# zeehu/generative_ranking_recommender

Measured on NVIDIA B200. Metric: RQ-KMeans vectors/sec per iteration (512-d, [128,128,256]), higher is better.
Workload: dtype 3xTF32 distance (fp32 accumulate), fp16 auction, fp32 centroids

## Files before the change

generative_ranking_recommender_b200/csrc/auction.cu:

```cuda
#include "common.cuh"

namespace rqk {

constexpr int AUC_W = 256;
constexpr int AUC_HALF = AUC_W / 2;
constexpr int AUC_NBUF = 3;
constexpr int AUC_BPL = AUC_W / 32;
constexpr int AUC_NW = 16;
constexpr int AUC_THREADS = AUC_NW * 32;
constexpr int AUC_BASE_CTAS = 296;
constexpr int AUC_MAX_CTAS = 1024;
constexpr int AUC_MAX_JOBS_PER_CTA = 65024;
constexpr int AUC_MIN_TILES_PER_CTA = 2;
constexpr int AUC_COLD_SHIFT = 8;
constexpr int AUC_MIN_KEY = 0x0400;
constexpr int AUC_SUB = 4096;
constexpr int AUC_QCAP = 256;
constexpr int AUC_SAMPLE_MAX = 8192;
constexpr int AUC_SEG_CAP = 256;
constexpr int AUC_KH = 128;
constexpr int AUC_SAMPLE_THREADS = 512;

enum { MODE_HIST = 0, MODE_BID = 1, MODE_DONE = 2 };

__device__ __forceinline__ void pdl_launch_dependents() { asm volatile("griddepcontrol.launch_dependents;" ::: "memory"); }
__device__ __forceinline__ void pdl_wait() { asm volatile("griddepcontrol.wait;" ::: "memory"); }

struct AuctionState {
    int mode;
    int counter;
    int rounds;
    int done;
    int ff_pending;
    int frozen_exit;
    int passes;
    int cold_passes;
    int window_misses;
    unsigned int eps_bits;
    unsigned int smax_bits, smin_bits;
    int need_sample;
    int error;
    int use_list;
    int force_scan;
    int list_passes;
    int sink[4];
    int branch[4];
    int pad_[4];
};

struct AuctionPtrs {
    AuctionState* st;
    __half* cost;
    short* owner;
    __half* sown;
    unsigned int* hist_g;
    unsigned int* above_g;
    unsigned int* gap_g;
    unsigned int* n_with;
    unsigned int* n_viol;
    unsigned int* tie_total;
    int* win_base;
    int* win_hbase;
    int* win_nlo;
    int* win_shift;
    int* tkey;
    int* take;
    int* tprev;
    int* miss_run;
    unsigned int* tieprefix;
    unsigned short* hist_cta;
    unsigned int* seg_list;
    unsigned int* seg_cnt;
    int* list_ok;
    unsigned int* rank_off;
    unsigned int* ticket;
    int* res_pass;
    unsigned int* above_cta;
    unsigned int* gap_cta;
    int* unres_g;
};

static inline int auction_tile_cols(int K) { return K <= 128 ? 128 : 64; }

static inline int auction_grid(long long N, int K) {
    long long tiles = ceil_div<long long>(N, auction_tile_cols(K));
    long long g = ceil_div<long long>(tiles, AUC_MIN_TILES_PER_CTA);
    const char* e = getenv("RQK_AUCTION_GRID");
    const int cap = (e && atoi(e) >= 1 && atoi(e) <= AUC_BASE_CTAS) ? atoi(e) : AUC_BASE_CTAS;
    if (g > cap) g = cap;
    long long g16 = ceil_div<long long>(N, AUC_MAX_JOBS_PER_CTA);
    if (g < g16) g = g16;
    if (g < 1) g = 1;
    return (int)g;
}

static inline int auction_spc(long long N, int K) {
    const int J = auction_tile_cols(K), G = auction_grid(N, K);
    const long long tiles = ceil_div<long long>(N, J);
    const long long len = ceil_div<long long>(tiles, G) * J;
    return (int)ceil_div<long long>(len, AUC_SUB);
}

static inline size_t auction_ws_layout(long long N, long long ld, int K, AuctionPtrs* p, char* base,
                                       size_t* reduce_off = nullptr, size_t* tie_total_off = nullptr) {
    int G = auction_grid(N, K);
    size_t off = 0;
    auto take_ = [&](size_t bytes) { size_t o = off; off += align256(bytes); return o; };
    size_t o_st = take_(sizeof(AuctionState));
    size_t o_cost = take_((size_t)ld * 2);
    size_t o_own = take_((size_t)ld * 2);
    size_t o_sown = take_((size_t)ld * 2);
    size_t o_hist = take_(((size_t)K * AUC_W + 2 * K + 2) * 4);
    size_t o_tt = take_((size_t)K * 4);
    size_t o_wb = take_((size_t)K * 4);
    size_t o_whb = take_((size_t)K * 4);
    size_t o_wnl = take_((size_t)K * 4);
    size_t o_ws = take_((size_t)K * 4);
    size_t o_tk = take_((size_t)K * 4);
    size_t o_take = take_((size_t)K * 4);
    size_t o_tprev = take_((size_t)K * 4);
    size_t o_mr = take_((size_t)K * 4);
    size_t o_tp = take_((size_t)G * K * 4);
    size_t o_hc = take_((size_t)G * K * AUC_W * 2);
    const size_t nseg = (size_t)G * auction_spc(N, K);
    size_t o_sl = take_(nseg * K * AUC_SEG_CAP * 4);
    size_t o_sc = take_(nseg * K * 4);
    size_t o_lo = take_(4);
    size_t o_ro = take_((size_t)K * 4);
    size_t o_tk2 = take_(4);
    size_t o_rp = take_((size_t)K * 4);
    size_t o_ac = take_((size_t)G * K * 4);
    size_t o_gc = take_((size_t)G * K * 4);
    size_t o_ug = take_(16);
    if (reduce_off) *reduce_off = o_hist;
    if (tie_total_off) *tie_total_off = o_tt;
    if (p) {
        p->st = (AuctionState*)(base + o_st);
        p->cost = (__half*)(base + o_cost);
        p->owner = (short*)(base + o_own);
        p->sown = (__half*)(base + o_sown);
        p->hist_g = (unsigned int*)(base + o_hist);
        p->above_g = p->hist_g + (size_t)K * AUC_W;
        p->gap_g = p->above_g + K;
        p->n_with = p->gap_g + K;
        p->n_viol = p->n_with + 1;
        p->tie_total = (unsigned int*)(base + o_tt);
        p->win_base = (int*)(base + o_wb);
        p->win_hbase = (int*)(base + o_whb);
        p->win_nlo = (int*)(base + o_wnl);
        p->win_shift = (int*)(base + o_ws);
        p->tkey = (int*)(base + o_tk);
        p->take = (int*)(base + o_take);
        p->tprev = (int*)(base + o_tprev);
        p->miss_run = (int*)(base + o_mr);
        p->tieprefix = (unsigned int*)(base + o_tp);
        p->hist_cta = (unsigned short*)(base + o_hc);
        p->seg_list = (unsigned int*)(base + o_sl);
        p->seg_cnt = (unsigned int*)(base + o_sc);
        p->list_ok = (int*)(base + o_lo);
        p->rank_off = (unsigned int*)(base + o_ro);
        p->ticket = (unsigned int*)(base + o_tk2);
        p->res_pass = (int*)(base + o_rp);
        p->above_cta = (unsigned int*)(base + o_ac);
        p->gap_cta = (unsigned int*)(base + o_gc);
        p->unres_g = (int*)(base + o_ug);
    }
    return off;
}

__global__ void auction_init_kernel(AuctionPtrs p, long long ld, int K, const unsigned int* minmax_keys, int force_scan) {
    long long i = (long long)blockIdx.x * blockDim.x + threadIdx.x;
    long long stride = (long long)gridDim.x * blockDim.x;
    for (long long j = i; j < ld; j += stride) {
        p.cost[j] = __ushort_as_half(0);
        p.owner[j] = -1;
    }
    for (long long j = i; j < (long long)K * AUC_W + 2 * K + 2; j += stride) p.hist_g[j] = 0;
    for (long long j = i; j < K; j += stride) {
        p.win_base[j] = 0;
        p.win_hbase[j] = AUC_HALF;
        p.win_nlo[j] = AUC_HALF;
        p.win_shift[j] = AUC_COLD_SHIFT;
        p.tkey[j] = -1;
        p.take[j] = 0;
        p.tprev[j] = -1;
        p.miss_run[j] = 0;
        p.rank_off[j] = 0;
        p.res_pass[j] = -1;
    }
    if (i == 0) {
        AuctionState s;
        memset(&s, 0, sizeof(s));
        s.mode = MODE_HIST;
        s.need_sample = 1;
        s.force_scan = force_scan;
        *p.list_ok = 1;
        *p.ticket = 0;
        p.unres_g[0] = 0;
// ... 139 lines not shown
        atomicAdd(&sink[5], 1);
        int nb2 = base + nlo, span = hbase - nb2, nshift = 0;
        while ((span >> nshift) > AUC_W) ++nshift;
        p.win_base[w] = nb2;
        p.win_hbase[w] = nb2 + AUC_HALF;
        p.win_nlo[w] = AUC_HALF;
        p.win_shift[w] = nshift;
        p.tkey[w] = -1;
        atomicAdd(unresolved, 1);
        atomicAdd(miss, 1);
    } else if (lane == 0) {
        const int run = p.miss_run[w];
        const bool is_above = ab >= (unsigned long long)need;
        int nb = is_above ? (shift == 0 ? hbase + (AUC_W - nlo) : base + (AUC_W << shift)) : base - (AUC_W << shift);
        atomicAdd(&sink[(shift != 0 || run >= 2 || nb < AUC_MIN_KEY || nb > 65536 - AUC_W) ? 7 : 6], 1);
        if (shift != 0 || run >= 2 || nb < AUC_MIN_KEY || nb > 65536 - AUC_W) {
            p.win_base[w] = 0;
            p.win_hbase[w] = AUC_HALF;
            p.win_nlo[w] = AUC_HALF;
            p.win_shift[w] = AUC_COLD_SHIFT;
            p.miss_run[w] = 0;
        } else {
            p.win_base[w] = nb;
            p.win_hbase[w] = nb + AUC_HALF;
            p.win_nlo[w] = AUC_HALF;
            p.miss_run[w] = run + 1;
        }
        p.tkey[w] = -1;
        atomicAdd(unresolved, 1);
        if (shift == 0) atomicAdd(miss, 1);
    }
}

__device__ __noinline__ void auction_resolve_body(AuctionPtrs p, long long N, int K, long long jpw, int expect) {
    __shared__ int s_unresolved, s_miss;
    __shared__ AuctionState s;
    __shared__ unsigned long long s_nwith_g, s_nviol_g;
    const int tid = threadIdx.x, lane = tid & 31, warp = tid >> 5;
    const int NT = blockDim.x, NWARPS = NT >> 5;
    if (tid == 0) { s = *p.st; s_unresolved = 0; s_miss = 0; s_nwith_g = *p.n_with; s_nviol_g = *p.n_viol; }
    __syncthreads();
    if (s.mode == MODE_DONE || (expect >= 0 && s.mode != expect)) return;
    const bool was_bid = (s.mode == MODE_BID);

    bool finished = false, jump = false;
    if (was_bid) {
        const BidOutcome o = bid_outcome(s.counter, s_nwith_g, s_nviol_g, N);
        finished = o.finished;
        jump = o.jump;
    }
    if (finished) {
        __syncthreads();
        if (tid == 0) {
            bool normal = (s_nwith_g == (unsigned long long)N);
            s.rounds = normal ? s.counter + 1 : 1002;
            s.frozen_exit = normal ? 0 : 1;
            s.mode = MODE_DONE;
            s.done = 1;
            s.passes += 1;
            if (s.use_list) s.list_passes += 1;
            *p.st = s;
        }
        return;
    }

    const long long need = jpw + 1;
    if (was_bid) {
// ... 9 lines not shown
        if (tid == 0) s_unresolved = 1;
    } else if (!jump) {
        unsigned int hn[AUC_BPL];
#pragma unroll
        for (int i = 0; i < AUC_BPL; ++i) hn[i] = (warp < K) ? __ldcg(p.hist_g + warp * AUC_W + lane * AUC_BPL + i) : 0u;
        for (int w = warp; w < K; w += NWARPS) {
            const bool settled = p.tkey[w] >= 0;
            const int base = p.win_base[w], shift = p.win_shift[w];
            const int hbase = p.win_hbase[w], nlo = (shift == 0) ? p.win_nlo[w] : 0;
            const unsigned long long gap = (shift == 0) ? p.gap_g[w] : 0ull;
            unsigned int h[AUC_BPL];
            unsigned int lsum = 0;
#pragma unroll
            for (int i = 0; i < AUC_BPL; ++i) { h[i] = hn[i]; lsum += h[i]; }
            if (w + NWARPS < K) {
#pragma unroll
                for (int i = 0; i < AUC_BPL; ++i) hn[i] = __ldcg(p.hist_g + (w + NWARPS) * AUC_W + lane * AUC_BPL + i);
            }
            if (settled) continue;
            resolve_one_worker(p, w, h, lsum, p.above_g[w], gap, base, shift, hbase, nlo, need, jpw, s.passes, s.sink,
                               &s_unresolved, &s_miss);
        }
    }
    __syncthreads();
    for (int i = tid + (was_bid ? K * AUC_W : 0); i < K * AUC_W + 2 * K + 2; i += NT) p.hist_g[i] = 0;
    __syncthreads();
    if (tid == 0) {
        s.passes += 1;
        if (!was_bid) s.cold_passes += 1;
        s.window_misses += s_miss;
        if (was_bid) s.counter += 1;
        s.ff_pending = 0;
        s.need_sample = was_bid ? 1 : 0;
        if (was_bid && s.use_list) s.list_passes += 1;
        if (!was_bid) s.use_list = (*p.list_ok != 0 && !s.force_scan) ? 1 : 0;
        else *p.list_ok = 1;
        if (jump) {
            s.ff_pending = 100 - s.counter;
            s.counter = 100;
            s.mode = MODE_HIST;
        } else {
            s.mode = (s_unresolved == 0) ? MODE_BID : MODE_HIST;
        }
        *p.st = s;
    }
}


__global__ void __launch_bounds__(1024, 1)
auction_resolve_kernel(AuctionPtrs p, long long N, int K, long long jpw, int expect) {
    auction_resolve_body(p, N, K, jpw, expect);
}

__device__ __forceinline__ bool auction_last_cta(unsigned int* ticket) {
    __shared__ int s_last;
    __threadfence();
    __syncthreads();
    if (threadIdx.x == 0) {
        const unsigned int t = atomicAdd(ticket, 1u);
        s_last = (t == gridDim.x - 1) ? 1 : 0;
        if (s_last) *ticket = 0;
    }
    __syncthreads();
    if (s_last) __threadfence();
    return s_last != 0;
}
// ... 692 lines not shown
                const unsigned int c = seg_cnt_s[tid];
                p.seg_cnt[(size_t)seg * K + tid] = c;
                if (c > AUC_SEG_CAP) *p.list_ok = 0;
            }
        }

        unsigned int* dump = reinterpret_cast<unsigned int*>(p.hist_cta + ((size_t)b * K + h0) * AUC_W);
        for (int a = tid >> 7; a < nact; a += AUC_THREADS >> 7) {
            const int i = ((int)acth[a] - h0) * (AUC_W / 2) + (tid & 127);
            const unsigned int h = sm.hist[i];
            dump[i] = h;
            if (!fused) {
                const int ig = h0 * (AUC_W / 2) + i;
                if (h & 0xffffu) atomicAdd(&p.hist_g[2 * ig], h & 0xffffu);
                if (h >> 16) atomicAdd(&p.hist_g[2 * ig + 1], h >> 16);
            }
        }
        ffh = 0;
    }

    const int nact_all = s_act_off[2];
    for (int a = tid; a < nact_all; a += AUC_THREADS) {
        const int i = act[a];
        if (fused) {
            p.above_cta[(size_t)b * K + i] = sm.above[i];
            p.gap_cta[(size_t)b * K + i] = sm.gap[i];
        } else {
            if (sm.above[i]) atomicAdd(&p.above_g[i], sm.above[i]);
            if (sm.gap[i]) atomicAdd(&p.gap_g[i], sm.gap[i]);
        }
    }
}

__global__ void __launch_bounds__(AUC_THREADS, 2)
auction_bidlist_kernel(const __half* __restrict__ S, long long ld, long long N, int K, int J, int spc, AuctionPtrs p,
                       long long n_global, int fused) {
    pdl_launch_dependents();
    pdl_wait();
    const AuctionState st = *p.st;
    if (st.mode != MODE_BID || !st.use_list) return;
    constexpr int NCH = AUC_SEG_CAP / 32;
    __shared__ __align__(16) unsigned int colmax[AUC_SUB];
    __shared__ __align__(16) short own_s[AUC_SUB];
    __shared__ __align__(16) unsigned char colviol[AUC_SUB];
    __shared__ unsigned int tie_seen[256];
    __shared__ int r_take[256], r_tk[256];
    __shared__ unsigned int s_nwith, s_nviol;
    const int tid = threadIdx.x, lane = tid & 31, warp = tid >> 5;
    const int counter = st.counter;
    const __half eps = bits2h(st.eps_bits);
    const unsigned int eps_bits = st.eps_bits;
    const bool retain = counter >= 1 && counter < 100;
    const bool fallback = counter > 1000;
    const int G = gridDim.x, b = blockIdx.x;
    const long long tiles_total = (N + J - 1) / J;
    const long long c_begin = (tiles_total * b / G) * J;
    long long c_end = (tiles_total * (b + 1) / G) * J;
    if (c_end > N) c_end = N;

    for (int i = tid; i < K; i += AUC_THREADS) {
        tie_seen[i] = p.tieprefix[(size_t)b * K + i];
        r_tk[i] = p.tkey[i];
        r_take[i] = p.take[i];
    }
    if (tid == 0) { s_nwith = 0; s_nviol = 0; }

// ... 141 lines not shown
                unsigned int c = (cw[e >> 1] >> sh) & 0xffffu, o = (ow[e >> 1] >> sh) & 0xffffu;
                const int old_owner = (int)(short)o;
                bool vv = ((e < 4 ? vi.x >> (8 * e) : vi.y >> (8 * (e - 4))) & 0xffu) != 0;
                if (pk[e]) {
                    ++n_has;
                    c = h2bits(__hadd(__ushort_as_half((unsigned short)c), bits2h(pk[e] >> 16)));
                    cost_dirty = true;
                    if ((changed >> e) & 1u) { o = 0xffffu - (pk[e] & 0xffffu); own_dirty = true; }
                } else if (old_owner >= 0) {
                    o = 0xffffu;
                    own_dirty = true;
                    vv = true;
                }
                n_vv += vv ? 1 : 0;
                if (e & 1) { nc[e >> 1] |= c << 16; no[e >> 1] |= o << 16; }
                else { nc[e >> 1] = c; no[e >> 1] = o; }
            }
            if (grp) {
                if (cost_dirty) *reinterpret_cast<uint4*>(p.cost + sub + j0) = make_uint4(nc[0], nc[1], nc[2], nc[3]);
                if (own_dirty) *reinterpret_cast<uint4*>(p.owner + sub + j0) = make_uint4(no[0], no[1], no[2], no[3]);
#pragma unroll
                for (int e = 0; e < 8; ++e)
                    if ((changed >> e) & 1u) p.sown[sub + j0 + e] = __ushort_as_half(sv[e]);
            }
            n_has = __reduce_add_sync(0xffffffffu, n_has);
            n_vv = __reduce_add_sync(0xffffffffu, n_vv);
            if (lane == 0) {
                if (n_has) atomicAdd(&s_nwith, (unsigned)n_has);
                if (n_vv) atomicAdd(&s_nviol, (unsigned)n_vv);
            }
        }
        __syncthreads();
    }
    if (tid == 0) {
        if (s_nwith) atomicAdd(p.n_with, s_nwith);
        if (s_nviol) atomicAdd(p.n_viol, s_nviol);
    }
    if (fused && auction_last_cta(p.ticket)) auction_resolve_body(p, n_global, K, n_global / K, MODE_BID);
}

static inline size_t auction_pass_smem(int K, int J) {
    return (size_t)AUC_NBUF * K * J * 2 + (size_t)K * 16 + (size_t)J * 4 +
           (size_t)J * 4 + (size_t)K * 2 + (size_t)J + 64;
}

constexpr int AUC_SAMPLE = AUC_SAMPLE_MAX;
__device__ __forceinline__ void sample_select_bin(const unsigned int* hist, int base, int need, int* out_bin, int* out_above) {
    const int lane = threadIdx.x & 31;
    int h[8], lsum = 0;
#pragma unroll
    for (int i = 0; i < 8; ++i) { h[i] = (int)hist[lane * 8 + i]; lsum += h[i]; }
    int suf = lsum;
#pragma unroll
    for (int d = 1; d < 32; d <<= 1) {
        const int o = __shfl_down_sync(0xffffffffu, suf, d);
        if (lane + d < 32) suf += o;
    }
    int c = base + suf - lsum, bin = -1, above = 0;
#pragma unroll
    for (int i = 7; i >= 0; --i) {
        if (bin < 0 && c + h[i] >= need) { bin = lane * 8 + i; above = c; }
        c += h[i];
    }
    const unsigned int who = __ballot_sync(0xffffffffu, bin >= 0);
    int rb = 0, ra = base + __shfl_sync(0xffffffffu, suf, 0);
    if (who) {
        const int src = 31 - __clz(who);
        rb = __shfl_sync(0xffffffffu, bin, src);
        ra = __shfl_sync(0xffffffffu, above, src);
    }
    if (lane == 0) { *out_bin = rb; *out_above = ra; }
    *out_bin = rb;
    *out_above = ra;
}



__global__ void __launch_bounds__(AUC_SAMPLE_THREADS, 2)
auction_sample_kernel(const __half* __restrict__ S, long long ld, long long N, int K, long long jpw, AuctionPtrs p,
                      unsigned short* __restrict__ collect_out, int collect_n,
                      const unsigned short* __restrict__ ext_keys, int ext_n, int ext_cnt, PeerCtx peers, int peer_seq) {
    pdl_launch_dependents();
    pdl_wait();
    const AuctionState st = *p.st;
    if (st.mode != MODE_HIST || !st.need_sample) return;
    __shared__ unsigned short keys[AUC_SAMPLE];
    const int w = blockIdx.x, tid = threadIdx.x;
    if (peers.world > 0) {
        if (!peer_barrier(peers, 0, peer_seq, blockIdx.x == 0)) {
            if (tid == 0) { p.st->error = 1; p.st->mode = MODE_DONE; p.st->done = 1; }
            return;
        }
    }
    long long ns = N < AUC_SAMPLE ? N : AUC_SAMPLE;
    if (collect_out) ns = collect_n < ns ? collect_n : ns;
    if (ext_keys || peers.world > 0) ns = ext_n;
    const __half eps = bits2h(st.eps_bits);
    {
        constexpr int PER = 8;
        static_assert(AUC_SAMPLE % (PER * AUC_SAMPLE_THREADS) == 0, "whole batches");
        const long long nchunks = (ns + 15) / 16, cstride = N / (nchunks > 0 ? nchunks : 1);
        for (int q0 = 0; q0 < AUC_SAMPLE / AUC_SAMPLE_THREADS; q0 += PER) {
            __half c_r[PER], s_r[PER];
            short o_r[PER];
            unsigned short k_r[PER];
#pragma unroll
            for (int q = 0; q < PER; ++q) {
                const int i = tid + (q0 + q) * AUC_SAMPLE_THREADS;
                k_r[q] = 0;
                c_r[q] = s_r[q] = __ushort_as_half(0);
                o_r[q] = -1;
                if (ext_keys || peers.world > 0) {
                    if (i < ns) {
                        if (peers.world > 0)
                            k_r[q] = __ldcv(peer_sample(peers, i / ext_cnt, K, peer_seq & 1) + (size_t)w * ext_cnt + (i % ext_cnt));
                        else
                            k_r[q] = ext_keys[((size_t)(i / ext_cnt) * K + w) * ext_cnt + (i % ext_cnt)];
                    }
                } else if (i < ns) {
                    long long col = cstride * (i >> 4) + (i & 15);
                    if (col >= N) col = N - 1;
                    c_r[q] = p.cost[col];
                    o_r[q] = p.owner[col];
                    s_r[q] = S[(size_t)w * ld + col];
                }
            }
#pragma unroll
            for (int q = 0; q < PER; ++q) {
                const int i = tid + (q0 + q) * AUC_SAMPLE_THREADS;
                unsigned short key = k_r[q];
                if (!ext_keys && peers.world == 0 && i < ns) {
                    __half c = c_r[q];
                    if (st.ff_pending > 0 && o_r[q] >= 0)
                        for (int r = 0; r < st.ff_pending; ++r) c = __hadd(c, eps);
                    const __half v = (o_r[q] == w) ? s_r[q] : __hsub(s_r[q], c);
                    key = (unsigned short)h2key(h2bits(v));
                }
                keys[i] = key;
                if (collect_out && i < collect_n) collect_out[(size_t)w * collect_n + i] = key;
            }
        }
    }
    if (collect_out) return;
    __syncthreads();
    __shared__ unsigned int shist[256];
    __shared__ unsigned short top[1024], sorted[1024];
    __shared__ int s_b1, s_above1, s_vlo, s_cnt;
    bool need_full_sort = true;
    {
        const double r = (double)(jpw + 1) * (double)ns / (double)N - 0.5;
        const double sg = sqrt(r > 1.0 ? r : 1.0);
        long long r_lo = (long long)ceil(r + 4.5 * sg + 2.0);
        if (r_lo > ns - 1) r_lo = ns - 1;
        const int need_n = (int)r_lo + 1;
        if (need_n <= 512) {
            if (tid < 256) shist[tid] = 0;
            if (tid == 0) s_cnt = 0;
            __syncthreads();
            for (int i = tid; i < AUC_SAMPLE; i += AUC_SAMPLE_THREADS) atomicAdd(&shist[keys[i] >> 8], 1u);
            __syncthreads();
            if (tid < 32) sample_select_bin(shist, 0, need_n, &s_b1, &s_above1);
            __syncthreads();
            const int b1 = s_b1;
            if (tid < 256) shist[tid] = 0;
            __syncthreads();
            for (int i = tid; i < AUC_SAMPLE; i += AUC_SAMPLE_THREADS)
                if ((keys[i] >> 8) == b1) atomicAdd(&shist[keys[i] & 255], 1u);
            __syncthreads();
            if (tid < 32) {
                int bsel, dummy;
                sample_select_bin(shist, s_above1, need_n, &bsel, &dummy);
                if (tid == 0) s_vlo = (b1 << 8) | bsel;
            }
            __syncthreads();
            const int vlo = s_vlo;
            for (int i = tid; i < AUC_SAMPLE; i += AUC_SAMPLE_THREADS) {
                const unsigned short kk = keys[i];
                if ((int)kk >= vlo) {
                    const int slot = atomicAdd(&s_cnt, 1);
                    if (slot < 1024) top[slot] = kk;
                }
            }
            __syncthreads();
            const int cnt = s_cnt;
            if (cnt <= 1024) {
                need_full_sort = false;
                for (int i = tid; i < cnt; i += AUC_SAMPLE_THREADS) {
                    const unsigned short kk = top[i];
                    int rank = 0;
                    for (int j = 0; j < cnt; ++j) {
                        const unsigned short kj = top[j];
                        rank += (kj > kk) || (kj == kk && j < i);
                    }
                    sorted[rank] = kk;
                }
                __syncthreads();
                for (int i = tid; i < cnt; i += AUC_SAMPLE_THREADS) keys[i] = sorted[i];
                __syncthreads();
            }
        }
    }
    if (need_full_sort) {
        for (int k = 2; k <= AUC_SAMPLE; k <<= 1) {
            for (int j = k >> 1; j > 0; j >>= 1) {
                for (int i = tid; i < AUC_SAMPLE; i += AUC_SAMPLE_THREADS) {
                    const int ixj = i ^ j;
                    if (ixj > i) {
                        const unsigned short a = keys[i], b2 = keys[ixj];
                        const bool desc = (i & k) == 0;
                        if (desc ? (a < b2) : (a > b2)) { keys[i] = b2; keys[ixj] = a; }
                    }
                }
                __syncthreads();
            }
        }
    }
    if (tid == 0) {
        const double r = (double)(jpw + 1) * (double)ns / (double)N - 0.5;
        const double sg = sqrt(r > 1.0 ? r : 1.0);
        long long r_hi = (long long)floor(r - 4.5 * sg - 2.0), r_lo = (long long)ceil(r + 4.5 * sg + 2.0);
        if (r_hi < 0) r_hi = 0;
        if (r_lo > ns - 1) r_lo = ns - 1;
        int lo = (int)keys[r_lo] - 1, hi = (int)keys[r_hi] + 1;
        if (r_hi == 0) hi += 32;
        const int tp = p.tprev[w];
        if (tp >= 0 && hi > tp + 2) hi = tp + 2;
        if (lo < AUC_MIN_KEY) lo = AUC_MIN_KEY;
        if (hi < lo + 8) hi = lo + 8;
        if (hi > 65535) hi = 65535;
        int span = hi - lo + 1, shift = 0, hb = lo + AUC_HALF, nlo = AUC_HALF;
        if (span > AUC_W) {
            long long cut = -1;
            int hole = 0;
            for (long long q = r_hi; q < r_lo; ++q) {
                const int d = (int)keys[q] - (int)keys[q + 1];
                if (d > hole) { hole = d; cut = q; }
            }
            bool ok = false;
            if (cut >= 0) {
                const int up_lo = keys[cut], dn_hi = keys[cut + 1];
                const int need_up = hi - up_lo + 1, need_dn = dn_hi - lo + 1;
                if (need_up + need_dn <= AUC_W && need_up >= 1 && need_dn >= 1) {
                    int spare = AUC_W - need_up - need_dn;
                    const int room = up_lo - dn_hi - 1;
                    if (spare > room) spare = room;
                    const int ext_dn = spare / 2, ext_up = spare - ext_dn;
                    nlo = need_dn + ext_dn;
                    hb = up_lo - ext_up;
                    ok = true;
// ... 474 lines not shown
    if (k < 1 || k > 256) return fail(RQK_ERR_UNSUPPORTED, "%s: k=%lld outside [1,256]", who, k);
    if (n < 1) return fail(RQK_ERR_ARG, "%s: n=%lld < 1", who, n);
    if (ld % 128 != 0 || ld < n) return fail(RQK_ERR_ARG, "%s: ld=%lld must be a multiple of 128 and >= n", who, ld);
    size_t need = auction_ws_layout(n, ld, k, &a->p, (char*)workspace);
    if (workspace_bytes < need) return fail(RQK_ERR_WORKSPACE, "%s: workspace %lld < %lld bytes", who, (long long)workspace_bytes, (long long)need);
    a->G = auction_grid(n, k);
    if (a->G > AUC_MAX_CTAS) return fail(RQK_ERR_UNSUPPORTED, "%s: n=%lld jobs per GPU exceed the 66 M limit of this build", who, n);
    a->J = auction_tile_cols(k);
    a->smem = auction_pass_smem(k, a->J);
    return 0;
}

template <typename... KArgs, typename... Args>
static cudaError_t launch_round_kernel(void (*kernel)(KArgs...), unsigned grid, unsigned block, size_t smem,
                                       cudaStream_t stream, bool pdl, Args... args) {
    cudaLaunchConfig_t cfg = {};
    cfg.gridDim = dim3(grid);
    cfg.blockDim = dim3(block);
    cfg.dynamicSmemBytes = smem;
    cfg.stream = stream;
    cudaLaunchAttribute attr[1];
    attr[0].id = cudaLaunchAttributeProgrammaticStreamSerialization;
    attr[0].val.programmaticStreamSerializationAllowed = 1;
    cfg.attrs = attr;
    cfg.numAttrs = pdl ? 1 : 0;
    return cudaLaunchKernelEx(&cfg, kernel, KArgs(args)...);
}

static bool auction_list_refine_ok() {
    static const bool ok = [] { const char* e = getenv("RQK_AUCTION_NO_LIST_REFINE"); return !(e && e[0] == '1'); }();
    return ok;
}

static bool auction_pdl_ok() {
    static const bool ok = [] { const char* e = getenv("RQK_NO_PDL"); return !(e && e[0] == '1'); }();
    return ok;
}

static int auction_launch(const AuctionArgs& a, const void* scores_t, int64_t ld, int64_t n, int32_t k, int64_t n_global,
                          int which, int fused, cudaStream_t stream, bool chain = false) {
    const bool pdl = (fused != 0 || chain) && auction_pdl_ok();
    auto kern = (a.J == 128) ? auction_pass_kernel<128> : auction_pass_kernel<64>;
    int devi = 0;
    RQK_CUDA_OK(cudaGetDevice(&devi));
    devi &= RQK_MAX_DEVICES - 1;
    static size_t smem_set[RQK_MAX_DEVICES][2] = {};
    size_t& cur = smem_set[devi][a.J == 128 ? 0 : 1];
    if (a.smem > cur) {
        RQK_CUDA_OK(cudaFuncSetAttribute(kern, cudaFuncAttributeMaxDynamicSharedMemorySize, (int)a.smem));
        cur = a.smem;
    }
    const int spc = auction_spc(n, k);
    if (which & 1)
        RQK_CUDA_OK(launch_round_kernel(auction_sample_kernel, (unsigned)k, (unsigned)AUC_SAMPLE_THREADS, 0, stream, pdl, (const __half*)scores_t,
                                        (long long)ld, (long long)n, (int)k, (long long)(n_global / k), a.p,
                                        (unsigned short*)nullptr, 0, (const unsigned short*)nullptr, 0, 1, PeerCtx{}, 0));
    if (which & 2) {
        static bool hs_set[RQK_MAX_DEVICES] = {};
        const size_t hs = HistSmem::TOTAL;
        if (!hs_set[devi]) {
            RQK_CUDA_OK(cudaFuncSetAttribute(auction_hist_kernel, cudaFuncAttributeMaxDynamicSharedMemorySize, (int)hs));
            hs_set[devi] = true;
        }
        RQK_CUDA_OK(launch_round_kernel(auction_hist_kernel, (unsigned)a.G, (unsigned)AUC_THREADS, hs, stream, pdl,
                                        (const __half*)scores_t, (long long)ld, (long long)n, (int)k, a.J, spc, a.p,
                                        (long long)n_global, fused));
    }
    if (which & 8)
        RQK_CUDA_OK(launch_round_kernel(auction_merge_resolve_kernel, (unsigned)k, (unsigned)AUC_MAX_CTAS, 0, stream, pdl,
                                        a.p, (int)k, a.G, (long long)(n_global / k), spc, auction_list_refine_ok() ? 1 : 0));
    if (which & 4) {
        RQK_CUDA_OK(launch_round_kernel(auction_bidlist_kernel, (unsigned)a.G, (unsigned)AUC_THREADS, 0, stream, pdl,
                                        (const __half*)scores_t, (long long)ld, (long long)n, (int)k, a.J, spc, a.p,
                                        (long long)n_global, fused));
        RQK_CUDA_OK(launch_round_kernel(kern, (unsigned)a.G, (unsigned)AUC_THREADS, a.smem, stream, pdl,
                                        (const __half*)scores_t, (long long)ld, (long long)n, (int)k, (long long)(n_global / k),
                                        a.p, (long long)n_global, fused));
    }
    RQK_LAUNCH_OK();
    return 0;
}
}

extern "C" {

struct rqk_auction_layout {
    int64_t total_bytes;
    int64_t reduce_offset;
    int64_t reduce_count;
// ... 37 lines not shown
    if (rc) return rc;
    if (!minmax_keys) return fail(RQK_ERR_ARG, "rqk_auction_init: null minmax_keys%s");
    cudaStream_t stream = (cudaStream_t)stream_;
    RQK_CUDA_OK(cudaMemsetAsync(a.p.tieprefix, 0, (size_t)a.G * k * 4, stream));
    const char* ns = getenv("RQK_AUCTION_NO_LIST");
    auction_init_kernel<<<148, 256, 0, stream>>>(a.p, ld, k, (const unsigned int*)minmax_keys, (ns && ns[0] == '1') ? 1 : 0);
    RQK_LAUNCH_OK();
    return 0;
}

int rqk_auction_pass(const void* scores_t, int64_t ld, int64_t n, int32_t k, int64_t n_global, int32_t which,
                     void* workspace, size_t workspace_bytes, void* stream_) {
    using namespace rqk;
    AuctionArgs a;
    int rc = auction_prepare(n, ld, k, workspace, workspace_bytes, &a, "rqk_auction_pass");
    if (rc) return rc;
    if (!scores_t) return fail(RQK_ERR_ARG, "rqk_auction_pass: null scores%s");
    if (n_global < k) return fail(RQK_ERR_ARG, "rqk_auction_pass: n_global=%s%lld < k=%lld (argmin path, reference :24-26)", "", n_global, k);
    if (which == 0) which = 7;
    if (n_global != n) which &= ~1;
    const int fused = (which & 16) && n_global == n ? 1 : 0;
    if ((which & 8) && !fused) return fail(RQK_ERR_ARG, "rqk_auction_pass: bit 3 (merge + resolve) needs bit 4 and unsharded jobs%s");
    return auction_launch(a, scores_t, ld, n, k, n_global, which & 15, fused, (cudaStream_t)stream_);
}

int rqk_auction_sample_collect(const void* scores_t, int64_t ld, int64_t n, int32_t k, int64_t n_global, void* out,
                               int32_t count, void* workspace, size_t workspace_bytes, void* stream_) {
    using namespace rqk;
    AuctionArgs a;
    int rc = auction_prepare(n, ld, k, workspace, workspace_bytes, &a, "rqk_auction_sample_collect");
    if (rc) return rc;
    if (!scores_t || !out || count < 1 || count > AUC_SAMPLE) return fail(RQK_ERR_ARG, "rqk_auction_sample_collect: bad argument%s");
    auction_sample_kernel<<<k, AUC_SAMPLE_THREADS, 0, (cudaStream_t)stream_>>>((const __half*)scores_t, ld, n, k, n_global / k, a.p,
                                                                  (unsigned short*)out, count, nullptr, 0, 1, PeerCtx{}, 0);
    RQK_LAUNCH_OK();
    return 0;
}

int rqk_auction_sample_window(int64_t n, int64_t ld, int32_t k, int64_t n_global, const void* keys, int32_t count,
                              int32_t parts, void* workspace, size_t workspace_bytes, void* stream_) {
    using namespace rqk;
    AuctionArgs a;
    int rc = auction_prepare(n, ld, k, workspace, workspace_bytes, &a, "rqk_auction_sample_window");
    if (rc) return rc;
    if (!keys || count < 1 || parts < 1 || (int64_t)count * parts > AUC_SAMPLE)
        return fail(RQK_ERR_ARG, "rqk_auction_sample_window: bad argument%s");
    auction_sample_kernel<<<k, AUC_SAMPLE_THREADS, 0, (cudaStream_t)stream_>>>(nullptr, ld, n_global, k, n_global / k, a.p, nullptr, 0,
                                                                  (const unsigned short*)keys, count * parts, count, PeerCtx{}, 0);
    RQK_LAUNCH_OK();
    return 0;
}

int rqk_auction_resolve(int64_t n, int64_t ld, int32_t k, int64_t n_global, int32_t expect, void* workspace,
                        size_t workspace_bytes, void* stream_) {
    using namespace rqk;
    AuctionArgs a;
    int rc = auction_prepare(n, ld, k, workspace, workspace_bytes, &a, "rqk_auction_resolve");
    if (rc) return rc;
    cudaStream_t stream = (cudaStream_t)stream_;
    if (expect < -1 || expect > 1) return fail(RQK_ERR_ARG, "rqk_auction_resolve: expect must be -1, 0 or 1%s");
    auction_resolve_kernel<<<1, 1024, 0, stream>>>(a.p, n_global, k, n_global / k, expect);
    auction_tieprefix_kernel<<<k, AUC_MAX_CTAS, 0, stream>>>(a.p, k, a.G);
    RQK_LAUNCH_OK();
    return 0;
}

size_t rqk_auction_peer_bytes(int32_t k) { return rqk::peer_bytes(k); }

static int peer_ctx(const void* const* peers, int32_t world, int32_t rank, rqk::PeerCtx* c, const char* who) {
    using namespace rqk;
    if (!peers || world < 1 || world > PEER_MAX || rank < 0 || rank >= world)
        return fail(RQK_ERR_ARG, "%s: bad peer arguments (world 1..8)", who);
    for (int r = 0; r < PEER_MAX; ++r) c->buf[r] = r < world ? (unsigned char*)peers[r] : nullptr;
    for (int r = 0; r < world; ++r)
        if (!c->buf[r]) return fail(RQK_ERR_ARG, "%s: null peer pointer", who);
    c->world = world;
    c->rank = rank;
    return 0;
}

int rqk_auction_peer_round(const void* scores_t, int64_t ld, int64_t n, int32_t k, int64_t n_global, int32_t count,
                           const void* const* peers, int32_t world, int32_t rank, int32_t seq0, void* workspace,
                           size_t workspace_bytes, void* stream_) {
    using namespace rqk;
    AuctionArgs a;
    int rc = auction_prepare(n, ld, k, workspace, workspace_bytes, &a, "rqk_auction_peer_round");
    if (rc) return rc;
    PeerCtx c;
    if ((rc = peer_ctx(peers, world, rank, &c, "rqk_auction_peer_round"))) return rc;
    if (!scores_t || count < 1 || (int64_t)count * world > AUC_SAMPLE) return fail(RQK_ERR_ARG, "rqk_auction_peer_round: bad argument%s");
    if (n_global < k) return fail(RQK_ERR_ARG, "rqk_auction_peer_round: n_global=%s%lld < k=%lld", "", n_global, k);
    cudaStream_t stream = (cudaStream_t)stream_;
    const bool pdl = auction_pdl_ok();
    RQK_CUDA_OK(launch_round_kernel(auction_peer_bid_collect_kernel, (unsigned)k, 1024u, 0, stream, pdl, (const __half*)scores_t,
                                    (long long)ld, (long long)n, (int)k, (long long)n_global, a.p, (int)count, c, (int)seq0,
                                    (int)(seq0 + 1)));
    RQK_CUDA_OK(launch_round_kernel(auction_sample_kernel, (unsigned)k, (unsigned)AUC_SAMPLE_THREADS, 0, stream, pdl, (const __half*)nullptr, (long long)ld,
                                    (long long)n_global, (int)k, (long long)(n_global / k), a.p, (unsigned short*)nullptr, 0,
                                    (const unsigned short*)nullptr, (int)(count * world), (int)count, c, (int)(seq0 + 1)));
    if ((rc = auction_launch(a, scores_t, ld, n, k, n_global, 2, 1, stream, true))) return rc;
    RQK_CUDA_OK(launch_round_kernel(auction_peer_publish_kernel, (unsigned)k, (unsigned)AUC_MAX_CTAS, 0, stream, pdl, a.p, (int)k,
                                    a.G, c, (int)(seq0 + 2)));
    RQK_CUDA_OK(launch_round_kernel(auction_peer_resolve_workers_kernel, (unsigned)k, (unsigned)AUC_MAX_CTAS, 0, stream, pdl, a.p,
                                    (int)k, a.G, (long long)(n_global / k), c, (int)(seq0 + 2)));
    if ((rc = auction_launch(a, scores_t, ld, n, k, n_global, 4, 0, stream, true))) return rc;
    RQK_LAUNCH_OK();
    return 0;
}

int rqk_auction_tie_offset(int64_t n, int64_t ld, int32_t k, const int32_t* totals, int32_t rank, void* workspace,
                           size_t workspace_bytes, void* stream_) {
    using namespace rqk;
    AuctionArgs a;
    int rc = auction_prepare(n, ld, k, workspace, workspace_bytes, &a, "rqk_auction_tie_offset");
    if (rc) return rc;
    if (!totals || rank < 0) return fail(RQK_ERR_ARG, "rqk_auction_tie_offset: bad argument%s");
    if (rank == 0) return 0;
    auction_tie_offset_kernel<<<ceil_div(a.G * k, 256), 256, 0, (cudaStream_t)stream_>>>(a.p, k, a.G, totals, rank);
    RQK_LAUNCH_OK();
    return 0;
}

int rqk_auction_poll(int64_t n, int64_t ld, int32_t k, void* workspace, size_t workspace_bytes, rqk_auction_info* info,
                     void* stream_) {
    using namespace rqk;
    AuctionArgs a;
    int rc = auction_prepare(n, ld, k, workspace, workspace_bytes, &a, "rqk_auction_poll");
    if (rc) return rc;
    if (!info) return fail(RQK_ERR_ARG, "rqk_auction_poll: null info%s");
    AuctionState host;
    cudaStream_t stream = (cudaStream_t)stream_;
    RQK_CUDA_OK(cudaMemcpyAsync(&host, a.p.st, sizeof(host), cudaMemcpyDeviceToHost, stream));
// ... 38 lines not shown
    cudaStream_t stream = (cudaStream_t)stream_;
    static thread_local AuctionState* mailbox_d[RQK_MAX_DEVICES] = {};
    static thread_local cudaEvent_t ev_d[RQK_MAX_DEVICES][2];
    int devi = 0;
    RQK_CUDA_OK(cudaGetDevice(&devi));
    devi &= RQK_MAX_DEVICES - 1;
    if (!mailbox_d[devi]) {
        RQK_CUDA_OK(cudaHostAlloc((void**)&mailbox_d[devi], 2 * sizeof(AuctionState), cudaHostAllocPortable));
        RQK_CUDA_OK(cudaEventCreateWithFlags(&ev_d[devi][0], cudaEventDisableTiming));
        RQK_CUDA_OK(cudaEventCreateWithFlags(&ev_d[devi][1], cudaEventDisableTiming));
    }
    AuctionState* mailbox = mailbox_d[devi];
    cudaEvent_t* ev = ev_d[devi];
    const int rounds_per_batch = 2;
    const AuctionState* fin = nullptr;
    for (int b = 0; b < 4000 && !fin; ++b) {
        for (int q = 0; q < rounds_per_batch; ++q)
            if ((rc = auction_launch(a, scores_t, ld, n, k, n, 1 | 2 | 4 | 8, 1, stream))) return rc;
        RQK_CUDA_OK(cudaMemcpyAsync(&mailbox[b & 1], a.p.st, sizeof(AuctionState), cudaMemcpyDeviceToHost, stream));
        RQK_CUDA_OK(cudaEventRecord(ev[b & 1], stream));
        if (b >= 1) {
            RQK_CUDA_OK(cudaEventSynchronize(ev[(b - 1) & 1]));
            if (mailbox[(b - 1) & 1].done) fin = &mailbox[(b - 1) & 1];
        }
    }
    RQK_CUDA_OK(cudaStreamSynchronize(stream));
    if (fin) {
        st.done = fin->done; st.rounds = fin->rounds; st.passes = fin->passes; st.cold_passes = fin->cold_passes;
        st.window_misses = fin->window_misses; st.frozen_exit = fin->frozen_exit; st.counter = fin->counter;
        st.eps_bits = (uint16_t)fin->eps_bits;
        st.list_passes = (uint16_t)(fin->list_passes > 65535 ? 65535 : fin->list_passes);
    }
    if (fin) {
        static const bool dbg = [] { const char* e = getenv("RQK_AUCTION_DEBUG"); return e && e[0] == '1'; }();
        if (dbg)
            fprintf(stderr, "rqk_auction n=%lld k=%d: rounds %d passes %d (HIST %d, from lists %d) window misses %d | worker-passes: "
                    "refine in coarse bin %d, in gap %d, slide %d, coarse restart %d | sink <64 %d <128 %d <250 %d >=250 %d\n",
                    (long long)n, (int)k, fin->rounds, fin->passes, fin->cold_passes, fin->list_passes, fin->window_misses,
                    fin->branch[0], fin->branch[1], fin->branch[2], fin->branch[3], fin->sink[0], fin->sink[1], fin->sink[2],
                    fin->sink[3]);
    }
    if (!st.done) return fail(RQK_ERR_INTERNAL, "rqk_auction: did not terminate%s");
    if ((rc = rqk_auction_finalize(n, ld, k, workspace, workspace_bytes, assign, stream_))) return rc;
    if (info) *info = st;
    return 0;
}

}
```

Before: 196.4 million.

## Stage auction sample keys in fused bid kernel and replace sample sort with radix select

The fused bid-list kernel now computes each worker's sampled price keys after bidding and writes them to a global staging buffer. The sample kernel then loads them with vector loads instead of re-gathering cost, owner and score values. The sample kernel's partial/bitonic sort is replaced by a two-level histogram radix select that extracts only the needed rank window. This cuts scattered gathers and sort work on the sample path, at the cost of extra workspace, extra work at the end of the bid kernel, and a debug-only verification path.

```diff
diff --git a/generative_ranking_recommender_b200/csrc/auction.cu b/generative_ranking_recommender_b200/csrc/auction.cu
--- a/generative_ranking_recommender_b200/csrc/auction.cu
+++ b/generative_ranking_recommender_b200/csrc/auction.cu
@@ -45,7 +45,10 @@
     int list_passes;
     int sink[4];
     int branch[4];
-    int pad_[4];
+    int keys_staged;
+    int stage_checked;
+    int stage_mismatch;
+    int pad_;
 };
 
 struct AuctionPtrs {
@@ -78,6 +81,7 @@
     unsigned int* above_cta;
     unsigned int* gap_cta;
     int* unres_g;
+    unsigned short* sample_keys;
 };
 
 static inline int auction_tile_cols(int K) { return K <= 128 ? 128 : 64; }
@@ -132,6 +136,7 @@
     size_t o_ac = take_((size_t)G * K * 4);
     size_t o_gc = take_((size_t)G * K * 4);
     size_t o_ug = take_(16);
+    size_t o_sk = take_((size_t)K * AUC_SAMPLE_MAX * 2);
     if (reduce_off) *reduce_off = o_hist;
     if (tie_total_off) *tie_total_off = o_tt;
     if (p) {
@@ -164,6 +169,7 @@
         p->above_cta = (unsigned int*)(base + o_ac);
         p->gap_cta = (unsigned int*)(base + o_gc);
         p->unres_g = (int*)(base + o_ug);
+        p->sample_keys = (unsigned short*)(base + o_sk);
     }
     return off;
 }
@@ -369,7 +375,8 @@
     }
 }
 
-__device__ __noinline__ void auction_resolve_body(AuctionPtrs p, long long N, int K, long long jpw, int expect) {
+__device__ __noinline__ void auction_resolve_body(AuctionPtrs p, long long N, int K, long long jpw, int expect,
+                                                  int staged = 0) {
     __shared__ int s_unresolved, s_miss;
     __shared__ AuctionState s;
     __shared__ unsigned long long s_nwith_g, s_nviol_g;
@@ -445,6 +452,7 @@
         if (was_bid) s.counter += 1;
         s.ff_pending = 0;
         s.need_sample = was_bid ? 1 : 0;
+        s.keys_staged = (was_bid && staged && !jump) ? 1 : 0;
         if (was_bid && s.use_list) s.list_passes += 1;
         if (!was_bid) s.use_list = (*p.list_ok != 0 && !s.force_scan) ? 1 : 0;
         else *p.list_ok = 1;
@@ -1203,6 +1211,47 @@
     }
 }
 
+__device__ __noinline__ void bidlist_stage_sample(const __half* __restrict__ S, long long ld, long long N, int K, int J,
+                                                  const __half* cost, const short* owner, unsigned short* sample_keys) {
+    const long long tiles_total = (N + J - 1) / J;
+    const long long c_begin = (tiles_total * blockIdx.x / gridDim.x) * J;
+    long long c_end = (tiles_total * (blockIdx.x + 1) / gridDim.x) * J;
+    if (c_end > N) c_end = N;
+    if (c_begin >= c_end) return;
+    const long long ns = N < AUC_SAMPLE_MAX ? N : AUC_SAMPLE_MAX;
+    const long long nchunks = (ns + 15) / 16, cstride = N / nchunks;
+    const long long ch0 = c_begin <= 15 ? 0 : (c_begin - 15 + cstride - 1) / cstride;
+    long long ch1 = (c_end - 1) / cstride;
+    if (ch1 > nchunks - 1) ch1 = nchunks - 1;
+    const int items = ch1 >= ch0 ? (int)(ch1 - ch0 + 1) * K * 16 : 0;
+    constexpr int PER = 6;
+    for (int t0 = threadIdx.x; t0 < items; t0 += PER * blockDim.x) {
+        __half c_r[PER], s_r[PER];
+        short o_r[PER];
+        int i_r[PER];
+#pragma unroll
+        for (int q = 0; q < PER; ++q) {
+            const int t = t0 + q * blockDim.x, tq = t >> 4, wk = tq % K;
+            const int i = (int)(ch0 + tq / K) * 16 + (t & 15);
+            long long col = cstride * (i >> 4) + (i & 15);
+            if (col >= N) col = N - 1;
+            i_r[q] = (t < items && i < ns && col >= c_begin && col < c_end) ? i : -1;
+            if (i_r[q] >= 0) {
+                c_r[q] = cost[col];
+                o_r[q] = owner[col];
+                s_r[q] = S[(size_t)wk * ld + col];
+            }
+        }
+#pragma unroll
+        for (int q = 0; q < PER; ++q) {
+            if (i_r[q] < 0) continue;
+            const int wk = ((t0 + q * (int)blockDim.x) >> 4) % K;
+            sample_keys[(size_t)wk * AUC_SAMPLE_MAX + i_r[q]] =
+                (unsigned short)h2key(h2bits((o_r[q] == wk) ? s_r[q] : __hsub(s_r[q], c_r[q])));
+        }
+    }
+}
+
 __global__ void __launch_bounds__(AUC_THREADS, 2)
 auction_bidlist_kernel(const __half* __restrict__ S, long long ld, long long N, int K, int J, int spc, AuctionPtrs p,
                        long long n_global, int fused) {
@@ -1410,11 +1459,12 @@
         }
         __syncthreads();
     }
+    if (fused) bidlist_stage_sample(S, ld, N, K, J, p.cost, p.owner, p.sample_keys);
     if (tid == 0) {
         if (s_nwith) atomicAdd(p.n_with, s_nwith);
         if (s_nviol) atomicAdd(p.n_viol, s_nviol);
     }
-    if (fused && auction_last_cta(p.ticket)) auction_resolve_body(p, n_global, K, n_global / K, MODE_BID);
+    if (fused && auction_last_cta(p.ticket)) auction_resolve_body(p, n_global, K, n_global / K, MODE_BID, 1);
 }
 
 static inline size_t auction_pass_smem(int K, int J) {
@@ -1423,47 +1473,19 @@
 }
 
 constexpr int AUC_SAMPLE = AUC_SAMPLE_MAX;
-__device__ __forceinline__ void sample_select_bin(const unsigned int* hist, int base, int need, int* out_bin, int* out_above) {
-    const int lane = threadIdx.x & 31;
-    int h[8], lsum = 0;
-#pragma unroll
-    for (int i = 0; i < 8; ++i) { h[i] = (int)hist[lane * 8 + i]; lsum += h[i]; }
-    int suf = lsum;
-#pragma unroll
-    for (int d = 1; d < 32; d <<= 1) {
-        const int o = __shfl_down_sync(0xffffffffu, suf, d);
-        if (lane + d < 32) suf += o;
-    }
-    int c = base + suf - lsum, bin = -1, above = 0;
-#pragma unroll
-    for (int i = 7; i >= 0; --i) {
-        if (bin < 0 && c + h[i] >= need) { bin = lane * 8 + i; above = c; }
-        c += h[i];
-    }
-    const unsigned int who = __ballot_sync(0xffffffffu, bin >= 0);
-    int rb = 0, ra = base + __shfl_sync(0xffffffffu, suf, 0);
-    if (who) {
-        const int src = 31 - __clz(who);
-        rb = __shfl_sync(0xffffffffu, bin, src);
-        ra = __shfl_sync(0xffffffffu, above, src);
-    }
-    if (lane == 0) { *out_bin = rb; *out_above = ra; }
-    *out_bin = rb;
-    *out_above = ra;
-}
-
-
+constexpr int AUC_SEL_BINS = 16;
 
 __global__ void __launch_bounds__(AUC_SAMPLE_THREADS, 2)
 auction_sample_kernel(const __half* __restrict__ S, long long ld, long long N, int K, long long jpw, AuctionPtrs p,
                       unsigned short* __restrict__ collect_out, int collect_n,
-                      const unsigned short* __restrict__ ext_keys, int ext_n, int ext_cnt, PeerCtx peers, int peer_seq) {
+                      const unsigned short* __restrict__ ext_keys, int ext_n, int ext_cnt, PeerCtx peers, int peer_seq,
+                      int check) {
     pdl_launch_dependents();
     pdl_wait();
     const AuctionState st = *p.st;
     if (st.mode != MODE_HIST || !st.need_sample) return;
-    __shared__ unsigned short keys[AUC_SAMPLE];
-    const int w = blockIdx.x, tid = threadIdx.x;
+    __shared__ __align__(16) unsigned short keys[AUC_SAMPLE];
+    const int w = blockIdx.x, tid = threadIdx.x, lane = tid & 31, warp = tid >> 5;
     if (peers.world > 0) {
         if (!peer_barrier(peers, 0, peer_seq, blockIdx.x == 0)) {
             if (tid == 0) { p.st->error = 1; p.st->mode = MODE_DONE; p.st->done = 1; }
@@ -1474,10 +1496,26 @@
     if (collect_out) ns = collect_n < ns ? collect_n : ns;
     if (ext_keys || peers.world > 0) ns = ext_n;
     const __half eps = bits2h(st.eps_bits);
-    {
+    const bool staged = st.keys_staged && !collect_out && !ext_keys && peers.world == 0;
+    if (staged) {
+        const uint4* row = reinterpret_cast<const uint4*>(p.sample_keys + (size_t)w * AUC_SAMPLE);
+        for (int v = tid; v < AUC_SAMPLE / 8; v += AUC_SAMPLE_THREADS) {
+            uint4 q = __ldcg(row + v);
+            if (8 * v + 8 > ns) {
+                unsigned int* u = reinterpret_cast<unsigned int*>(&q);
+#pragma unroll
+                for (int e = 0; e < 8; ++e)
+                    if (8 * v + e >= ns) u[e >> 1] &= (e & 1) ? 0x0000ffffu : 0xffff0000u;
+            }
+            reinterpret_cast<uint4*>(keys)[v] = q;
+        }
+        __syncthreads();
+    }
+    if (!staged || check) {
         constexpr int PER = 8;
         static_assert(AUC_SAMPLE % (PER * AUC_SAMPLE_THREADS) == 0, "whole batches");
         const long long nchunks = (ns + 15) / 16, cstride = N / (nchunks > 0 ? nchunks : 1);
+        int differ = 0;
         for (int q0 = 0; q0 < AUC_SAMPLE / AUC_SAMPLE_THREADS; q0 += PER) {
             __half c_r[PER], s_r[PER];
             short o_r[PER];
@@ -1514,85 +1552,98 @@
                     const __half v = (o_r[q] == w) ? s_r[q] : __hsub(s_r[q], c);
                     key = (unsigned short)h2key(h2bits(v));
                 }
-                keys[i] = key;
+                if (staged) differ += keys[i] != key;
+                else keys[i] = key;
                 if (collect_out && i < collect_n) collect_out[(size_t)w * collect_n + i] = key;
             }
         }
+        if (staged) {
+            differ = __reduce_add_sync(0xffffffffu, differ);
+            if (lane == 0 && differ) atomicAdd(&p.st->stage_mismatch, differ);
+            if (tid == 0) atomicAdd(&p.st->stage_checked, 1);
+        }
     }
     if (collect_out) return;
     __syncthreads();
-    __shared__ unsigned int shist[256];
-    __shared__ unsigned short top[1024], sorted[1024];
-    __shared__ int s_b1, s_above1, s_vlo, s_cnt;
-    bool need_full_sort = true;
+    __shared__ unsigned int hist_hi[256], above_hi[256];
+    __shared__ __align__(16) unsigned int cnt[AUC_SEL_BINS * 256];
+    __shared__ unsigned int warp_sum[AUC_SAMPLE_THREADS / 32];
+    __shared__ unsigned short sel[1024];
+    __shared__ int s_bhi, s_blo;
+    int rk0, rk1;
     {
         const double r = (double)(jpw + 1) * (double)ns / (double)N - 0.5;
         const double sg = sqrt(r > 1.0 ? r : 1.0);
-        long long r_lo = (long long)ceil(r + 4.5 * sg + 2.0);
+        long long r_hi = (long long)floor(r - 4.5 * sg - 2.0), r_lo = (long long)ceil(r + 4.5 * sg + 2.0);
+        if (r_hi < 0) r_hi = 0;
         if (r_lo > ns - 1) r_lo = ns - 1;
-        const int need_n = (int)r_lo + 1;
-        if (need_n <= 512) {
-            if (tid < 256) shist[tid] = 0;
-            if (tid == 0) s_cnt = 0;
-            __syncthreads();
-            for (int i = tid; i < AUC_SAMPLE; i += AUC_SAMPLE_THREADS) atomicAdd(&shist[keys[i] >> 8], 1u);
-            __syncthreads();
-            if (tid < 32) sample_select_bin(shist, 0, need_n, &s_b1, &s_above1);
-            __syncthreads();
-            const int b1 = s_b1;
-            if (tid < 256) shist[tid] = 0;
-            __syncthreads();
-            for (int i = tid; i < AUC_SAMPLE; i += AUC_SAMPLE_THREADS)
-                if ((keys[i] >> 8) == b1) atomicAdd(&shist[keys[i] & 255], 1u);
-            __syncthreads();
-            if (tid < 32) {
-                int bsel, dummy;
-                sample_select_bin(shist, s_above1, need_n, &bsel, &dummy);
-                if (tid == 0) s_vlo = (b1 << 8) | bsel;
-            }
-            __syncthreads();
-            const int vlo = s_vlo;
-            for (int i = tid; i < AUC_SAMPLE; i += AUC_SAMPLE_THREADS) {
-                const unsigned short kk = keys[i];
-                if ((int)kk >= vlo) {
-                    const int slot = atomicAdd(&s_cnt, 1);
-                    if (slot < 1024) top[slot] = kk;
-                }
-            }
-            __syncthreads();
-            const int cnt = s_cnt;
-            if (cnt <= 1024) {
-                need_full_sort = false;
-                for (int i = tid; i < cnt; i += AUC_SAMPLE_THREADS) {
-                    const unsigned short kk = top[i];
-                    int rank = 0;
-                    for (int j = 0; j < cnt; ++j) {
-                        const unsigned short kj = top[j];
-                        rank += (kj > kk) || (kj == kk && j < i);
-                    }
-                    sorted[rank] = kk;
-                }
-                __syncthreads();
-                for (int i = tid; i < cnt; i += AUC_SAMPLE_THREADS) keys[i] = sorted[i];
-                __syncthreads();
-            }
-        }
-    }
-    if (need_full_sort) {
-        for (int k = 2; k <= AUC_SAMPLE; k <<= 1) {
-            for (int j = k >> 1; j > 0; j >>= 1) {
-                for (int i = tid; i < AUC_SAMPLE; i += AUC_SAMPLE_THREADS) {
-                    const int ixj = i ^ j;
-                    if (ixj > i) {
-                        const unsigned short a = keys[i], b2 = keys[ixj];
-                        const bool desc = (i & k) == 0;
-                        if (desc ? (a < b2) : (a > b2)) { keys[i] = b2; keys[ixj] = a; }
-                    }
-                }
-                __syncthreads();
-            }
-        }
-    }
+        rk0 = (int)(r_hi < r_lo ? r_hi : r_lo);
+        rk1 = (int)(r_hi < r_lo ? r_lo : r_hi);
+    }
+    if (tid < 256) hist_hi[tid] = 0;
+    __syncthreads();
+    for (int i = tid; i < AUC_SAMPLE; i += AUC_SAMPLE_THREADS) {
+        atomicAdd(&hist_hi[keys[i] >> 8], 1u);
+    }
+    __syncthreads();
+    if (warp == 0) {
+        unsigned int h[8], lsum = 0;
+#pragma unroll
+        for (int i = 0; i < 8; ++i) { h[i] = hist_hi[lane * 8 + i]; lsum += h[i]; }
+        unsigned int suf = lsum;
+#pragma unroll
+        for (int d = 1; d < 32; d <<= 1) {
+            const unsigned int o = __shfl_down_sync(0xffffffffu, suf, d);
+            if (lane + d < 32) suf += o;
+        }
+        unsigned int a = suf - lsum;
+#pragma unroll
+        for (int i = 7; i >= 0; --i) {
+            const int b = lane * 8 + i;
+            above_hi[b] = a;
+            if (a <= (unsigned)rk0 && (unsigned)rk0 < a + h[i]) s_bhi = b;
+            if (a <= (unsigned)rk1 && (unsigned)rk1 < a + h[i]) s_blo = b;
+            a += h[i];
+        }
+    }
+    __syncthreads();
+    const int b_lo = s_blo;
+    for (int gt = s_bhi; gt >= b_lo; gt -= AUC_SEL_BINS) {
+        const int top = (gt << 8) | 255;
+        for (int i = tid; i < AUC_SEL_BINS * 256; i += AUC_SAMPLE_THREADS) cnt[i] = 0;
+        __syncthreads();
+        for (int i = tid; i < AUC_SAMPLE; i += AUC_SAMPLE_THREADS) {
+            const int d = top - (int)keys[i];
+            if ((unsigned)d < (unsigned)(AUC_SEL_BINS * 256)) atomicAdd(&cnt[d], 1u);
+        }
+        __syncthreads();
+        static_assert(AUC_SEL_BINS * 256 == 8 * AUC_SAMPLE_THREADS, "8 counters per thread");
+        const uint4 ca = reinterpret_cast<const uint4*>(cnt)[2 * tid], cb = reinterpret_cast<const uint4*>(cnt)[2 * tid + 1];
+        const unsigned int c8[8] = {ca.x, ca.y, ca.z, ca.w, cb.x, cb.y, cb.z, cb.w};
+        unsigned int lsum = 0;
+#pragma unroll
+        for (int e = 0; e < 8; ++e) lsum += c8[e];
+        unsigned int incl = lsum;
+#pragma unroll
+        for (int d = 1; d < 32; d <<= 1) {
+            const unsigned int o = __shfl_up_sync(0xffffffffu, incl, d);
+            if (lane >= d) incl += o;
+        }
+        if (lane == 31) warp_sum[warp] = incl;
+        __syncthreads();
+        unsigned int rank = above_hi[gt] + incl - lsum;
+        for (int q = 0; q < warp; ++q) rank += warp_sum[q];
+#pragma unroll
+        for (int e = 0; e < 8; ++e) {
+            const int lo = (int)rank > rk0 ? (int)rank : rk0;
+            const int hi = (int)(rank + c8[e]) - 1 < rk1 ? (int)(rank + c8[e]) - 1 : rk1;
+            for (int q = lo; q <= hi; ++q) sel[q - rk0] = (unsigned short)(top - (8 * tid + e));
+            rank += c8[e];
+        }
+        __syncthreads();
+    }
+    for (int q = tid; q <= rk1 - rk0; q += AUC_SAMPLE_THREADS) keys[rk0 + q] = sel[q];
+    __syncthreads();
     if (tid == 0) {
         const double r = (double)(jpw + 1) * (double)ns / (double)N - 0.5;
         const double sg = sqrt(r > 1.0 ? r : 1.0);
@@ -2133,6 +2184,11 @@
     return ok;
 }
 
+static bool auction_debug() {
+    static const bool on = [] { const char* e = getenv("RQK_AUCTION_DEBUG"); return e && e[0] == '1'; }();
+    return on;
+}
+
 static bool auction_pdl_ok() {
     static const bool ok = [] { const char* e = getenv("RQK_NO_PDL"); return !(e && e[0] == '1'); }();
     return ok;
@@ -2155,7 +2211,8 @@
     if (which & 1)
         RQK_CUDA_OK(launch_round_kernel(auction_sample_kernel, (unsigned)k, (unsigned)AUC_SAMPLE_THREADS, 0, stream, pdl, (const __half*)scores_t,
                                         (long long)ld, (long long)n, (int)k, (long long)(n_global / k), a.p,
-                                        (unsigned short*)nullptr, 0, (const unsigned short*)nullptr, 0, 1, PeerCtx{}, 0));
+                                        (unsigned short*)nullptr, 0, (const unsigned short*)nullptr, 0, 1, PeerCtx{}, 0,
+                                        auction_debug() ? 1 : 0));
     if (which & 2) {
         static bool hs_set[RQK_MAX_DEVICES] = {};
         const size_t hs = HistSmem::TOTAL;
@@ -2259,7 +2316,7 @@
     if (rc) return rc;
     if (!scores_t || !out || count < 1 || count > AUC_SAMPLE) return fail(RQK_ERR_ARG, "rqk_auction_sample_collect: bad argument%s");
     auction_sample_kernel<<<k, AUC_SAMPLE_THREADS, 0, (cudaStream_t)stream_>>>((const __half*)scores_t, ld, n, k, n_global / k, a.p,
-                                                                  (unsigned short*)out, count, nullptr, 0, 1, PeerCtx{}, 0);
+                                                                  (unsigned short*)out, count, nullptr, 0, 1, PeerCtx{}, 0, 0);
     RQK_LAUNCH_OK();
     return 0;
 }
@@ -2273,7 +2330,7 @@
     if (!keys || count < 1 || parts < 1 || (int64_t)count * parts > AUC_SAMPLE)
         return fail(RQK_ERR_ARG, "rqk_auction_sample_window: bad argument%s");
     auction_sample_kernel<<<k, AUC_SAMPLE_THREADS, 0, (cudaStream_t)stream_>>>(nullptr, ld, n_global, k, n_global / k, a.p, nullptr, 0,
-                                                                  (const unsigned short*)keys, count * parts, count, PeerCtx{}, 0);
+                                                                  (const unsigned short*)keys, count * parts, count, PeerCtx{}, 0, 0);
     RQK_LAUNCH_OK();
     return 0;
 }
@@ -2324,7 +2381,7 @@
                                     (int)(seq0 + 1)));
     RQK_CUDA_OK(launch_round_kernel(auction_sample_kernel, (unsigned)k, (unsigned)AUC_SAMPLE_THREADS, 0, stream, pdl, (const __half*)nullptr, (long long)ld,
                                     (long long)n_global, (int)k, (long long)(n_global / k), a.p, (unsigned short*)nullptr, 0,
-                                    (const unsigned short*)nullptr, (int)(count * world), (int)count, c, (int)(seq0 + 1)));
+                                    (const unsigned short*)nullptr, (int)(count * world), (int)count, c, (int)(seq0 + 1), 0));
     if ((rc = auction_launch(a, scores_t, ld, n, k, n_global, 2, 1, stream, true))) return rc;
     RQK_CUDA_OK(launch_round_kernel(auction_peer_publish_kernel, (unsigned)k, (unsigned)AUC_MAX_CTAS, 0, stream, pdl, a.p, (int)k,
                                     a.G, c, (int)(seq0 + 2)));
@@ -2429,13 +2486,13 @@
         st.list_passes = (uint16_t)(fin->list_passes > 65535 ? 65535 : fin->list_passes);
     }
     if (fin) {
-        static const bool dbg = [] { const char* e = getenv("RQK_AUCTION_DEBUG"); return e && e[0] == '1'; }();
-        if (dbg)
+        if (auction_debug())
             fprintf(stderr, "rqk_auction n=%lld k=%d: rounds %d passes %d (HIST %d, from lists %d) window misses %d | worker-passes: "
-                    "refine in coarse bin %d, in gap %d, slide %d, coarse restart %d | sink <64 %d <128 %d <250 %d >=250 %d\n",
+                    "refine in coarse bin %d, in gap %d, slide %d, coarse restart %d | sink <64 %d <128 %d <250 %d >=250 %d | "
+                    "staged samples checked %d, keys differing %d\n",
                     (long long)n, (int)k, fin->rounds, fin->passes, fin->cold_passes, fin->list_passes, fin->window_misses,
                     fin->branch[0], fin->branch[1], fin->branch[2], fin->branch[3], fin->sink[0], fin->sink[1], fin->sink[2],
-                    fin->sink[3]);
+                    fin->sink[3], fin->stage_checked, fin->stage_mismatch);
     }
     if (!st.done) return fail(RQK_ERR_INTERNAL, "rqk_auction: did not terminate%s");
     if ((rc = rqk_auction_finalize(n, ld, k, workspace, workspace_bytes, assign, stream_))) return rc;
```

New measurement: 193.9 million, median of 6. -1.3%, worse.
